# patrikhuber/superviseddescent

Measured on NVIDIA H100. Metric: faces/sec RCR 22-landmark detect, higher is better.
Workload: dtype f32

## Files before the change

superviseddescent_b200/csrc/sd_hog.cu:

```cuda
#include "sd_internal.cuh"
#include "sd_hog_common.cuh"

#include <cmath>
#include <cuda_pipeline.h>

namespace {

constexpr int kHogThreads = 256;

struct HogArgs {
    const uint8_t* images;
    int width, height, row_stride;
    long long image_stride;
    int image_count;
    const int* image_index;
    const sd_roi* roi;
    const sd_frame* frames;
    uint8_t* roi_miss;
    const float* x;
    long long ldx;
    int N, L;
    int variant, nc, cs, K, fs, dd;
    const int* half;
    HogOrient orient;
    const int* rtab;
    const float* btab;
    int tma_count;
    float* A;
    long long ld;
    int* geometry;
    uint8_t* patches;
    int8_t* bins;
    int* status;
};

__device__ __forceinline__ int clip_index(int x, int a, int b) { return x >= a ? (x < b ? x : b - 1) : a; }
__device__ __forceinline__ short sat_short(int v) { return (short)(v > 32767 ? 32767 : (v < -32768 ? -32768 : v)); }

__global__ void hog_geometry_kernel(const float* __restrict__ x, long long ldx, int N, int L, const sd_eyes_dev eyes, float rel,
                                    int fixed_half, int fs, int* __restrict__ half_out, int* __restrict__ rtab, int* __restrict__ status)
{
    const int i = blockIdx.x;
    if (i >= N) return;
    __shared__ int s_half;
    if (threadIdx.x == 0) {
        bool degenerate;
        const int half = sd_patch_half(x + (long long)i * ldx, L, eyes, rel, fixed_half, &degenerate);
        if (degenerate) atomicOr(status, 1);
        half_out[i] = half;
        s_half = half;
    }
    __syncthreads();
    const int P = 2 * s_half;
    int* rt = rtab + (long long)i * 5 * fs;
    for (int t = threadIdx.x; t < fs; t += blockDim.x) {
        const double inv_scale = __ddiv_rn((double)fs, (double)P);
        const double scale = __ddiv_rn(1.0, inv_scale);
        float f = (float)__dadd_rn(__dmul_rn((double)t + 0.5, scale), -0.5);
        const int s = (int)floorf(f);
        f = __fsub_rn(f, (float)s);
        int sx = s;
        float fx = f;
        if (sx < 0) { fx = 0.f; sx = 0; }
        if (sx >= P - 1) { fx = 0.f; sx = P - 1; }
        const short2 xa = make_short2(sat_short(__float2int_rn(__fmul_rn(__fsub_rn(1.f, fx), 2048.f))),
                                      sat_short(__float2int_rn(__fmul_rn(fx, 2048.f))));
        const short2 yb = make_short2(sat_short(__float2int_rn(__fmul_rn(__fsub_rn(1.f, f), 2048.f))),
                                      sat_short(__float2int_rn(__fmul_rn(f, 2048.f))));
        rt[t] = sx;
        rt[fs + t] = *reinterpret_cast<const int*>(&xa);
        rt[2 * fs + t] = clip_index(s, 0, P);
        rt[3 * fs + t] = clip_index(s + 1, 0, P);
        rt[4 * fs + t] = *reinterpret_cast<const int*>(&yb);
    }
}

__global__ void hog_bintab_kernel(int fs, int nc, int cs, float* __restrict__ btab)
{
    __shared__ int s_sbin[256];
    for (int t = threadIdx.x; t < fs; t += blockDim.x) {
        int b;
        float w1, w2;
        hog_spatial_weight(t, cs, &b, &w1, &w2);
        s_sbin[t] = b;
        for (int c = 0; c < nc; ++c) btab[c * fs + t] = (b == c) ? w1 : ((b == c - 1) ? w2 : 0.f);
    }
    __syncthreads();
    int* lohi = reinterpret_cast<int*>(btab + nc * fs);
    for (int c = threadIdx.x; c < nc; c += blockDim.x) {
        int lo = fs, hi = -1;
        for (int t = 1; t <= fs - 2; ++t) {
            const int b = s_sbin[t];
            if (b == c || b == c - 1) { if (t < lo) lo = t; hi = t; }
        }
        lohi[c] = lo;
        lohi[nc + c] = hi;
    }
}

__device__ __forceinline__ int hog_resize_out(int yb, int t0, int t1)
{
    return (((((int)(short)yb) * (t0 >> 4)) >> 16) + (((yb >> 16) * (t1 >> 4)) >> 16) + 2) >> 2;
}

__device__ __forceinline__ int byte_of(unsigned lo, unsigned hi, int n) { return (int)(((n < 4 ? lo : hi) >> (8 * (n & 3))) & 0xffu); }

struct HogSmem {
    int patch, bin, r1, tab, xa, wcell, lo, hi, vote, mbar, stage_end, total;
    int pp;
    int pb, pm;
    int tpad;
};

__host__ __device__ inline int align_up(int v, int a) { return (v + a - 1) / a * a; }

__host__ __device__ inline HogSmem hog_smem_layout(int fs, int nc, int K)
{
    HogSmem s;
    s.pp = align_up(fs, 4);
    s.pm = align_up(fs - 2, 4) + 1;
    s.pb = s.pm - 1;
    if ((s.pb & 7) == 0 && (fs - 2) * (s.pb + 4) <= fs * fs) s.pb += 4;
    int o = 0;
    s.patch = o;
    o = align_up(s.pp * fs, 16);
    s.tab = o;    o += fs * 16;
    s.xa = o;     o += fs * 4;
    s.wcell = o;  o += nc * fs * 4;
    s.lo = o;     o += nc * 4;
    s.hi = o;     o += nc * 4;
    s.mbar = align_up(o, 8); o = s.mbar + 8;
    o = align_up(o, 128);
    s.bin = o;    o = align_up(o + fs * fs, 16);
    s.r1 = o;     o = align_up(o + fs * fs * 4, 16);
    s.tpad = align_up((fs - 2) * nc, 32);
    s.vote = o;
    o += 2 * K * s.tpad * 4;
    s.stage_end = o;
    s.total = align_up(o + 8, 16);
    return s;
}

constexpr int kTmaClasses = 8;
__host__ __device__ constexpr int hog_tma_box(int c) { return c == 0 ? 32 : c == 1 ? 48 : c == 2 ? 64 : c == 3 ? 80 : c == 4 ? 96 : c == 5 ? 112 : c == 6 ? 128 : 160; }
struct HogMaps { CUtensorMap m[kTmaClasses]; };

template <int KT, int NCT, int CST, int NT>
__global__ void __launch_bounds__(NT, NCT > 0 ? 2048 / NT : 0) hog_patch_kernel(const __grid_constant__ HogArgs a, const __grid_constant__ HogMaps maps)
{
    static_assert(NT % 32 == 0 && NT >= 64, "hog_patch_kernel needs whole warps and at least 64 threads");
    constexpr int kWarps = NT / 32;
    extern __shared__ __align__(128) unsigned char smem[];
    const int K = KT > 0 ? KT : a.K;
    const int nc = NCT > 0 ? NCT : a.nc;
    const int fs = (NCT > 0 && CST > 0) ? NCT * CST : a.fs;
    const int cells = nc * nc;
    const HogSmem lay = hog_smem_layout(fs, nc, K);
    const int pp = lay.pp, pb = lay.pb, pm = lay.pm;
    uint8_t* s_patch = smem + lay.patch;
    int8_t* s_bin = reinterpret_cast<int8_t*>(smem + lay.bin);
    float* s_gmag = reinterpret_cast<float*>(smem + lay.r1);
    int4* s_tab = reinterpret_cast<int4*>(smem + lay.tab);
    short2* s_xa = reinterpret_cast<short2*>(smem + lay.xa);
    float* s_wcell = reinterpret_cast<float*>(smem + lay.wcell);
    int* s_lo = reinterpret_cast<int*>(smem + lay.lo);
    int* s_hi = reinterpret_cast<int*>(smem + lay.hi);
    float* s_T = reinterpret_cast<float*>(smem + lay.vote);
    uint64_t* s_mbar = reinterpret_cast<uint64_t*>(smem + lay.mbar);

    const int tid = threadIdx.x;
    const int lane = tid & 31, warp = tid >> 5;
    const long long patch_id = blockIdx.x;
    const int sample = (int)(patch_id / a.L);
    const int lm = (int)(patch_id - (long long)sample * a.L);

    const float* __restrict__ row = a.x + (long long)sample * a.ldx;
    const int half = __ldg(a.half + sample);
    const int P = 2 * half;
    const int cx = __float2int_rn(row[lm]);
    const int cy = __float2int_rn(row[lm + a.L]);
    int img_idx = a.image_index ? a.image_index[sample] : sample;
    if (img_idx < 0 || img_idx >= a.image_count) {
        img_idx = 0;
        if (tid == 0 && a.status) atomicOr(a.status, 2);
    }
    int W = a.width, H = a.height, rs = a.row_stride;
    const uint8_t* __restrict__ img = a.images + (long long)img_idx * a.image_stride;
    if (a.frames) {
        const sd_frame f = a.frames[img_idx];
        W = f.width; H = f.height; rs = f.row_stride;
        img = a.images + f.offset;
    }
    int rx = 0, ry = 0, rw = W, rh = H;
    if (a.roi) {
        const sd_roi r = a.roi[img_idx];
        rx = r.x; ry = r.y; rw = r.w; rh = r.h; rs = r.row_stride;
        img = a.images + r.offset;
    }
    if (tid == 0 && a.geometry) {
        a.geometry[patch_id * 3 + 0] = cx;
        a.geometry[patch_id * 3 + 1] = cy;
        a.geometry[patch_id * 3 + 2] = half;
    }

    const int x0 = cx - half, y0 = cy - half;
    uint8_t* s_stage = smem + lay.bin;
    const int stage_cap = lay.stage_end - lay.bin;
    int tma_box = 0;
    const int tma_shift = x0 & 15;
#pragma unroll
    for (int c = kTmaClasses - 1; c >= 0; --c)
        if (c < a.tma_count && hog_tma_box(c) >= P + tma_shift && hog_tma_box(c) * hog_tma_box(c) <= stage_cap) tma_box = hog_tma_box(c);
    if (tma_box > 0 && tid == 0) {
        int cls = 0;
#pragma unroll
        for (int c = 0; c < kTmaClasses; ++c) if (hog_tma_box(c) == tma_box) cls = c;
        hog_tma_load(s_mbar, s_stage, &maps.m[cls], x0 - tma_shift, y0, img_idx, tma_box * tma_box);
    }

    {
        const int* __restrict__ rt = a.rtab + (long long)sample * 5 * fs;
        for (int t = tid; t < fs; t += NT) {
            const int xa = __ldg(rt + fs + t);
            s_xa[t] = *reinterpret_cast<const short2*>(&xa);
            s_tab[t] = make_int4(__ldg(rt + t), __ldg(rt + 2 * fs + t), __ldg(rt + 3 * fs + t), __ldg(rt + 4 * fs + t));
        }
        for (int i = tid; i < nc * fs; i += NT) s_wcell[i] = __ldg(a.btab + i);
        const int* __restrict__ lohi = reinterpret_cast<const int*>(a.btab + nc * fs);
        if (tid < nc) { s_lo[tid] = __ldg(lohi + tid); s_hi[tid] = __ldg(lohi + nc + tid); }
    }
    {
        const bool resident = x0 >= rx && y0 >= ry && x0 + P <= rx + rw && y0 + P <= ry + rh && x0 >= 0 && y0 >= 0 && x0 + P <= W && y0 + P <= H;
        const uintptr_t align_bits = reinterpret_cast<uintptr_t>(img) | (uintptr_t)rs;
        const bool vec16 = !tma_box && resident && (align_bits & 15) == 0;
        const bool words = !tma_box && resident && (align_bits & 3) == 0;
        const int shiftb = tma_box ? tma_shift : (vec16 ? ((x0 - rx) & 15) : (words ? ((x0 - rx) & 3) : 0));
        const int pitch = tma_box ? tma_box : ((P + 15 + 15) & ~15);
        const bool staged = pitch * P <= stage_cap;
        bool miss = false;
        if (staged) {
            if (tma_box) {
            } else if (vec16) {
                const int nvec = (shiftb + P + 15) >> 4;
                const int gs = nvec <= 8 ? 3 : (nvec <= 16 ? 4 : 5);
                const int lv = lane & ((1 << gs) - 1), lr = lane >> gs, rows_per_pass = 32 >> gs;
                const uint8_t* wrow = img + (long long)(y0 - ry) * rs + (x0 - rx - shiftb);
                for (int r = warp * rows_per_pass + lr; r < P; r += kWarps * rows_per_pass)
#pragma unroll 1
                    for (int v = lv; v < nvec; v += (1 << gs))
                        reinterpret_cast<uint4*>(s_stage + r * pitch)[v] = __ldg(reinterpret_cast<const uint4*>(wrow + (long long)r * rs) + v);
            } else if (words) {
                const int nwords = (shiftb + P + 3) >> 2;
                const uint8_t* wrow = img + (long long)(y0 - ry) * rs + (x0 - rx - shiftb);
                for (int r = warp; r < P; r += kWarps) {
                    const uint32_t* src = reinterpret_cast<const uint32_t*>(wrow + (long long)r * rs);
                    uint32_t* dst = reinterpret_cast<uint32_t*>(s_stage + r * pitch);
#pragma unroll 1
                    for (int w = lane; w < nwords; w += 32) dst[w] = __ldg(src + w);
                }
            } else {
                for (int r = warp; r < P; r += kWarps) {
                    const int iy = y0 + r;
                    const bool rowin = (unsigned)iy < (unsigned)H;
                    const bool rowres = iy >= ry && iy < ry + rh;
                    for (int c = lane; c < P; c += 32) {
                        const int ix = x0 + c;
                        int v = 0;
                        if (rowin && (unsigned)ix < (unsigned)W) {
                            if (rowres && ix >= rx && ix < rx + rw) v = __ldg(img + (long long)(iy - ry) * rs + (ix - rx));
                            else miss = true;
                        }
                        s_stage[r * pitch + c] = (uint8_t)v;
                    }
                }
            }
            __syncthreads();
            if (tma_box) hog_tma_wait(s_mbar);
            if (fs <= 64) {
                const int np = (fs + 1) >> 1, groups = NT / np;
                const int j = tid % np, g = tid / np;
                if (g < groups) {
                    const int dxa = 2 * j, dxb = min(dxa + 1, fs - 1);
                    const int sxa = s_tab[dxa].x, sxb = s_tab[dxb].x;
                    const unsigned xa = *reinterpret_cast<const unsigned*>(s_xa + dxa), xb = *reinterpret_cast<const unsigned*>(s_xa + dxb);
                    const int q = (shiftb + sxa) & ~3;
                    const int oa = shiftb + sxa - q, ob = shiftb + sxb - q;
                    uint8_t* out = s_patch + dxa;
                    if (ob <= 6) {
                        const unsigned sa = oa | (oa + 1) << 4, sb = ob | (ob + 1) << 4;
                        const uint8_t* base = s_stage + q;
#pragma unroll 2
                        for (int dy = g; dy < fs; dy += groups) {
                            const int4 yt = s_tab[dy];
                            const unsigned* r0 = reinterpret_cast<const unsigned*>(base + yt.y * pitch);
                            const unsigned* r1 = reinterpret_cast<const unsigned*>(base + yt.z * pitch);
                            const unsigned a0 = r0[0], a1 = r0[1], b0 = r1[0], b1 = r1[1];
                            const int va = hog_resize_out(yt.w, __dp2a_lo(xa, __byte_perm(a0, a1, sa), 0u), __dp2a_lo(xa, __byte_perm(b0, b1, sa), 0u));
                            const int vb = hog_resize_out(yt.w, __dp2a_lo(xb, __byte_perm(a0, a1, sb), 0u), __dp2a_lo(xb, __byte_perm(b0, b1, sb), 0u));
                            *reinterpret_cast<uint16_t*>(out + dy * pp) = (uint16_t)(va | vb << 8);
                        }
                    } else {
                        const int ax = s_xa[dxa].x, bx = s_xa[dxa].y, cx = s_xa[dxb].x, dx = s_xa[dxb].y;
                        const int sxa1 = min(sxa + 1, P - 1), sxb1 = min(sxb + 1, P - 1);
                        const uint8_t* base = s_stage + shiftb;
                        for (int dy = g; dy < fs; dy += groups) {
                            const int4 yt = s_tab[dy];
                            const uint8_t* r0 = base + yt.y * pitch;
                            const uint8_t* r1 = base + yt.z * pitch;
                            const int va = hog_resize_out(yt.w, (int)r0[sxa] * ax + (int)r0[sxa1] * bx, (int)r1[sxa] * ax + (int)r1[sxa1] * bx);
                            const int vb = hog_resize_out(yt.w, (int)r0[sxb] * cx + (int)r0[sxb1] * dx, (int)r1[sxb] * cx + (int)r1[sxb1] * dx);
                            *reinterpret_cast<uint16_t*>(out + dy * pp) = (uint16_t)(va | vb << 8);
                        }
                    }
                }
            } else {
                for (int dy = warp; dy < fs; dy += kWarps) {
                    const int4 yt = s_tab[dy];
                    const uint8_t* r0 = s_stage + yt.y * pitch + shiftb;
                    const uint8_t* r1 = s_stage + yt.z * pitch + shiftb;
                    for (int dx = lane; dx < fs; dx += 32) {
                        const int sx = s_tab[dx].x;
                        const int sx1 = min(sx + 1, P - 1);
                        const short2 xa = s_xa[dx];
                        const int t0 = (int)r0[sx] * xa.x + (int)r0[sx1] * xa.y;
                        const int t1 = (int)r1[sx] * xa.x + (int)r1[sx1] * xa.y;
                        s_patch[dy * pp + dx] = (uint8_t)hog_resize_out(yt.w, t0, t1);
                    }
                }
            }
        } else {
            __syncthreads();
            for (int dy = warp; dy < fs; dy += kWarps) {
                const int4 yt = s_tab[dy];
                const int iy0 = y0 + yt.y, iy1 = y0 + yt.z;
                for (int dx = lane; dx < fs; dx += 32) {
                    const int sx = s_tab[dx].x;
                    const short2 xa = s_xa[dx];
                    int p[4];
#pragma unroll
                    for (int q = 0; q < 4; ++q) {
                        const int ix = x0 + sx + (q & 1), iy = (q & 2) ? iy1 : iy0;
                        int v = 0;
                        if ((q & 1) && xa.y == 0) { p[q] = 0; continue; }
                        if ((unsigned)ix < (unsigned)W && (unsigned)iy < (unsigned)H) {
                            if (ix >= rx && ix < rx + rw && iy >= ry && iy < ry + rh) v = __ldg(img + (long long)(iy - ry) * rs + (ix - rx));
                            else miss = true;
                        }
                        p[q] = v;
                    }
                    const int t0 = p[0] * xa.x + p[1] * xa.y;
                    const int t1 = p[2] * xa.x + p[3] * xa.y;
                    s_patch[dy * pp + dx] = (uint8_t)hog_resize_out(yt.w, t0, t1);
                }
            }
        }
        if (miss && a.roi_miss) a.roi_miss[img_idx] = 1;
        if (a.patches) {
            __syncthreads();
            for (int i = tid; i < fs * fs; i += NT) {
                const int y = i / fs;
                a.patches[patch_id * fs * fs + i] = s_patch[y * pp + (i - y * fs)];
            }
        }
    }
    __syncthreads();

    {
        const int iw = fs - 2, runs = (iw + 3) >> 2, nitem = iw * runs;
        const int pw = pp >> 2;
        for (int i = tid; i < nitem; i += NT) {
            const int y = i / runs, r = i - y * runs;
            const unsigned* c = reinterpret_cast<const unsigned*>(s_patch) + (y + 1) * pw + r;
            const unsigned c0 = c[0], c1 = c[1], u0 = c[-pw], u1 = c[1 - pw], d0 = c[pw], d1 = c[pw + 1];
            unsigned bins = 0;
            float* gm = s_gmag + y * pm + 4 * r;
#pragma unroll
            for (int k = 0; k < 4; ++k) {
                const int gx = byte_of(c0, c1, k + 2) - byte_of(c0, c1, k);
                const int gy = byte_of(d0, d1, k + 1) - byte_of(u0, u1, k + 1);
                const int g2 = gx * gx + gy * gy;
                const float g = __fsqrt_rn((float)g2);
                const int b = hog_bin(a.orient, K, gx, gy, g);
                bins |= (unsigned)(b & 0xff) << (8 * k);
                gm[k] = b < 0 ? 0.f : g;
            }
            *reinterpret_cast<unsigned*>(s_bin + y * pb + 4 * r) = bins;
        }
    }
    if (a.bins) {
        __syncthreads();
        for (int idx = tid; idx < fs * fs; idx += NT) {
            const int y = idx / fs, x = idx - y * fs;
            const bool interior = x >= 1 && x <= fs - 2 && y >= 1 && y <= fs - 2;
            a.bins[patch_id * fs * fs + idx] = interior ? s_bin[(y - 1) * pb + x - 1] : (int8_t)-1;
        }
    }
    if (!a.A) return;
    __syncthreads();

    {
        const int nrow = fs - 2, ntask = nrow * nc, tpad = lay.tpad;
        for (int task = tid; task < ntask; task += NT) {
            const int ci = task / nrow, y = 1 + task - ci * nrow;
            const int xlo = s_lo[ci], xhi = s_hi[ci];
            const int8_t* bp = s_bin + (y - 1) * pb + (xlo - 1);
            const float* gp = s_gmag + (y - 1) * pm + (xlo - 1);
            const float* wp = s_wcell + ci * fs + xlo;
            float* T = s_T + task;
            for (int b = 0; b < 2 * K; ++b) T[b * tpad] = 0.f;
#pragma unroll 2
            for (int x = xlo; x <= xhi; ++x) {
                const int b = max((int)*bp++, 0);
                float* q = T + b * tpad;
                *q = __fadd_rn(*q, __fmul_rn(*gp++, *wp++));
            }
        }
        __syncthreads();
        float* __restrict__ out = a.A + (long long)sample * a.ld + (long long)lm * cells * a.dd;
        for (int i = tid; i < 2 * K * cells; i += NT) {
            const int b = i / cells, c = i - b * cells;
            const int cj = c / nc, ci = c - cj * nc;
            const int ylo = s_lo[cj], yhi = s_hi[cj];
            const float* Tp = s_T + b * tpad + ci * nrow + (ylo - 1);
            const float* wy = s_wcell + cj * fs + ylo;
            float acc = 0.f;
            for (int y = ylo; y <= yhi; ++y) acc = __fadd_rn(acc, __fmul_rn(*Tp++, *wy++));
            out[i] = acc;
        }
    }
}

struct NormArgs {
    float* A;
    long long ld;
    int N, L, nc, K, dd, variant, per_cta;
};

__host__ __device__ inline int hog_norm_smem(int nc, int K, int per_cta)
{
    const int cells = nc * nc;
    return per_cta * (8 + 2 * K * cells * 4 + cells * 8 + (nc + 1) * (nc + 1) * 8);
}

template <int KT>
__global__ void __launch_bounds__(kHogThreads) hog_normalise_kernel(const NormArgs a)
{
    extern __shared__ __align__(16) unsigned char s_norm[];
    const int K = KT > 0 ? KT : a.K;
    const int nc = a.nc, nb = nc + 1, cells = nc * nc, blocks = nb * nb, hsz = 2 * K * cells, per_lm = cells * a.dd;
    const long long first = (long long)blockIdx.x * a.per_cta;
    const int np = (int)min((long long)a.per_cta, (long long)a.N * a.L - first);
    long long* s_slice = reinterpret_cast<long long*>(s_norm);
    double* s_energy = reinterpret_cast<double*>(s_slice + a.per_cta);
    double* s_fac = s_energy + a.per_cta * cells;
    float* s_hist = reinterpret_cast<float*>(s_fac + a.per_cta * blocks);
    for (int p = threadIdx.x; p < np; p += kHogThreads) {
        const long long id = first + p;
        const int sample = (int)(id / a.L), lm = (int)(id - (long long)sample * a.L);
        s_slice[p] = (long long)sample * a.ld + (long long)lm * per_lm;
        if (lm == 0) a.A[(long long)sample * a.ld + (long long)a.L * per_lm] = 1.0f;
    }
    __syncthreads();
    for (int i = threadIdx.x; i < np * hsz; i += kHogThreads) {
        const int p = i / hsz;
        __pipeline_memcpy_async(s_hist + i, a.A + s_slice[p] + (i - p * hsz), sizeof(float));
    }
    __pipeline_commit();
    __pipeline_wait_prior(0);
    __syncthreads();
    for (int i = threadIdx.x; i < np * cells; i += kHogThreads) {
        const int p = i / cells, c = i - p * cells;
        s_energy[i] = (double)hog_cell_energy(s_hist + p * hsz + c, cells, K);
    }
    __syncthreads();
    for (int i = threadIdx.x; i < np * blocks; i += kHogThreads) {
        const int p = i / blocks, j = i - p * blocks;
        const int jy = j / nb, jx = j - jy * nb;
        s_fac[i] = hog_block_factor(s_energy + p * cells, nc, max(jx - 1, 0), min(jx, nc - 1), max(jy - 1, 0), min(jy, nc - 1));
    }
    __syncthreads();
    for (int i = threadIdx.x; i < np * cells; i += kHogThreads) {
        const int p = i / cells, c = i - p * cells;
        const int cj = c / nc, ci = c - cj * nc;
        const double* F = s_fac + p * blocks + cj * nb + ci;
        const double fac[4] = {F[0], F[1], F[nb], F[nb + 1]};
        float* __restrict__ out = a.A + s_slice[p] + ci * nc + cj;
        hog_cell_features(fac, s_hist + p * hsz + c, cells, K, a.variant, [=](int d, float v) { out[d * cells] = v; });
    }
}

int launch_hog(sd_ctx* ctx, const sd_image_batch* images, const int32_t* d_image_index, const float* d_x,
               int64_t ldx, int N, int L, const sd_normalisation* eyes, const sd_hog_param* p, float* d_A,
               int64_t ld, int32_t* d_geometry, uint8_t* d_patches, int8_t* d_bins)
{
    SD_REQUIRE(ctx, images && images->d_data && d_x && p, "null argument");
    SD_REQUIRE(ctx, N >= 0 && L >= 1, "bad sample / landmark count");
    SD_REQUIRE(ctx, p->variant == 0 || p->variant == 1, "unknown HOG variant");
    SD_REQUIRE(ctx, p->num_bins >= 1 && p->num_bins <= SD_MAX_BINS, "num_bins must be in [1,16]");
    SD_REQUIRE(ctx, p->num_cells >= 1 && p->cell_size >= 1, "bad cell configuration");
    const int fs = p->num_cells * p->cell_size;
    SD_REQUIRE(ctx, fs > 3 && fs <= 256, "resized patch must be 4..256 px (hog.c:545-546 asserts > 3)");
    SD_REQUIRE(ctx, (fs + p->cell_size / 2) / p->cell_size == p->num_cells, "hogWidth != num_cells");
    SD_REQUIRE(ctx, ldx >= 2 * L, "ldx < 2L");
    if (N == 0) return SD_OK;
    const bool fixed = !eyes || eyes->kind == 0;
    int fixed_half = 0;
    if (fixed) {
        fixed_half = p->num_cells * (p->cell_size / 2);
        SD_REQUIRE(ctx, 2 * fixed_half == fs, "the fixed-patch HogTransform needs an even cell_size (patch == num_cells * cell_size)");
    } else if (eyes->kind != 1) {
        return sd_fail(ctx, SD_ERR_INVALID, "unknown normalisation kind");
    }

    HogArgs a;
    sd_eyes_dev eyes_dev;
    memset(&eyes_dev, 0, sizeof(eyes_dev));
    int rc = fixed ? SD_OK : sd_eyes_to_dev(ctx, eyes, L, &eyes_dev);
    if (rc) return rc;
    a.images = images->d_data;
    a.width = images->width; a.height = images->height; a.row_stride = images->row_stride;
    a.image_stride = images->image_stride; a.image_count = images->count;
    a.image_index = d_image_index;
    a.roi = images->d_roi;
    a.roi_miss = images->d_roi_miss;
    a.frames = images->d_frames;
    if (!d_image_index) SD_REQUIRE(ctx, images->count >= N, "fewer images than samples and no image index");
    a.x = d_x; a.ldx = ldx; a.N = N; a.L = L;
    a.variant = p->variant; a.nc = p->num_cells; a.cs = p->cell_size; a.K = p->num_bins; a.fs = fs;
    a.dd = p->variant == 1 ? 3 * p->num_bins + 4 : 4 * p->num_bins;
    a.A = d_A; a.ld = ld;
    if (d_A) SD_REQUIRE(ctx, ld >= (int64_t)L * a.nc * a.nc * a.dd + 1, "ld < feature length");
    const HogSmem lay = hog_smem_layout(fs, a.nc, a.K);
    const int cells = a.nc * a.nc;
    NormArgs na;
    na.A = d_A; na.ld = ld; na.N = N; na.L = L; na.nc = a.nc; na.K = a.K; na.dd = a.dd; na.variant = a.variant;
    na.per_cta = cells < kHogThreads ? kHogThreads / cells : 1;
    const int norm_smem = hog_norm_smem(a.nc, a.K, na.per_cta);
    SD_REQUIRE(ctx, lay.total <= 227 * 1024 && norm_smem <= 227 * 1024, "HOG configuration needs more than 227 KB of shared memory");
    const long long blocks = (long long)N * L;
    SD_REQUIRE(ctx, blocks < 2147483647LL, "too many patches for one launch");
    a.geometry = d_geometry; a.patches = d_patches; a.bins = d_bins;
    a.status = reinterpret_cast<int*>(ctx->d_scratch) + 1;

    hog_orientations(a.K, a.orient);

    const size_t geom_bytes = (size_t)N * sizeof(int) + (size_t)N * 5 * fs * sizeof(int) + (size_t)(a.nc * fs + 2 * a.nc) * sizeof(float);
    int* d_half = (int*)sd_workspace(ctx, SD_WS_GEOM, geom_bytes);
    if (!d_half) return SD_ERR_CUDA;
    int* d_rtab = d_half + N;
    float* d_btab = reinterpret_cast<float*>(d_rtab + (size_t)N * 5 * fs);
    hog_geometry_kernel<<<N, 64, 0, ctx->stream>>>(d_x, ldx, N, L, eyes_dev, p->relative_patch_size, fixed_half, fs, d_half, d_rtab, a.status);
    SD_LAUNCH_CHECK(ctx, "hog_geometry_kernel");
    hog_bintab_kernel<<<1, 256, 0, ctx->stream>>>(fs, a.nc, a.cs, d_btab);
    SD_LAUNCH_CHECK(ctx, "hog_bintab_kernel");
    a.half = d_half;
    a.rtab = d_rtab;
    a.btab = d_btab;

    HogMaps maps;
    memset(&maps, 0, sizeof(maps));
    a.tma_count = 0;
    if (!images->d_roi && (images->image_stride % 16) == 0 && (images->count == 1 || images->image_stride > 0)) {
        for (int c = 0; c < kTmaClasses && hog_tma_box(c) <= 256; ++c) {
            if (!hog_frame_map(images, hog_tma_box(c), hog_tma_box(c), &maps.m[c])) break;
            a.tma_count = c + 1;
        }
    }

    auto kern = hog_patch_kernel<0, 0, 0, kHogThreads>;
    int threads = kHogThreads;
    if (a.K == 4) kern = hog_patch_kernel<4, 0, 0, kHogThreads>;
    else if (a.K == 9) kern = hog_patch_kernel<9, 0, 0, kHogThreads>;
    if (a.nc == 5 && (a.K == 4 || a.K == 9)) {
#define SD_HOG_PICK(KK, CC, TT) if (a.K == KK && a.cs == CC) { kern = hog_patch_kernel<KK, 5, CC, TT>; threads = TT; }
        SD_HOG_PICK(4, 11, 224) SD_HOG_PICK(4, 10, 160) SD_HOG_PICK(4, 8, 160) SD_HOG_PICK(4, 6, 128)
        SD_HOG_PICK(9, 11, 256) SD_HOG_PICK(9, 10, 160) SD_HOG_PICK(9, 8, 160) SD_HOG_PICK(9, 6, 128)
#undef SD_HOG_PICK
    }
    SD_CUDA(ctx, cudaFuncSetAttribute(kern, cudaFuncAttributeMaxDynamicSharedMemorySize, lay.total));
    kern<<<(unsigned)blocks, threads, lay.total, ctx->stream>>>(a, maps);
    SD_LAUNCH_CHECK(ctx, "hog_patch_kernel");
    if (!d_A) return SD_OK;
    auto norm = a.K == 4 ? hog_normalise_kernel<4> : a.K == 9 ? hog_normalise_kernel<9> : hog_normalise_kernel<0>;
    SD_CUDA(ctx, cudaFuncSetAttribute(norm, cudaFuncAttributeMaxDynamicSharedMemorySize, norm_smem));
    norm<<<(unsigned)sd_div_up(blocks, na.per_cta), kHogThreads, norm_smem, ctx->stream>>>(na);
    SD_LAUNCH_CHECK(ctx, "hog_normalise_kernel");
    return SD_OK;
}

}

namespace {
__global__ void bgr2gray_kernel(const uint8_t* __restrict__ bgr, int width, int height, long long srow, long long simg, int count,
                                uint8_t* __restrict__ gray, long long drow, long long dimg, int vec_ok)
{
    const int groups = (width + 3) >> 2;
    const long long total = (long long)count * height * groups;
    for (long long t = blockIdx.x * (long long)blockDim.x + threadIdx.x; t < total; t += (long long)gridDim.x * blockDim.x) {
        const int g = (int)(t % groups);
        const long long ry = t / groups;
        const int y = (int)(ry % height);
        const long long im = ry / height;
        const uint8_t* s = bgr + im * simg + (long long)y * srow + 12 * g;
        uint8_t* d = gray + im * dimg + (long long)y * drow + 4 * g;
        const int x0 = 4 * g;
        if (vec_ok && x0 + 4 <= width) {
            const uint32_t w0 = *reinterpret_cast<const uint32_t*>(s), w1 = *reinterpret_cast<const uint32_t*>(s + 4),
                           w2 = *reinterpret_cast<const uint32_t*>(s + 8);
            const uint32_t b0 = w0 & 255, g0 = (w0 >> 8) & 255, r0 = (w0 >> 16) & 255, b1 = w0 >> 24;
            const uint32_t g1 = w1 & 255, r1 = (w1 >> 8) & 255, b2 = (w1 >> 16) & 255, g2 = w1 >> 24;
            const uint32_t r2 = w2 & 255, b3 = (w2 >> 8) & 255, g3 = (w2 >> 16) & 255, r3 = w2 >> 24;
            const uint32_t y0 = sd_bgr_to_gray(b0, g0, r0), y1 = sd_bgr_to_gray(b1, g1, r1);
            const uint32_t y2 = sd_bgr_to_gray(b2, g2, r2), y3 = sd_bgr_to_gray(b3, g3, r3);
            *reinterpret_cast<uint32_t*>(d) = y0 | (y1 << 8) | (y2 << 16) | (y3 << 24);
        } else {
            for (int k = 0; k < 4 && x0 + k < width; ++k) d[k] = (uint8_t)sd_bgr_to_gray(s[3 * k], s[3 * k + 1], s[3 * k + 2]);
        }
    }
}
}

extern "C" {

int sd_hog_feature_length(int num_landmarks, const sd_hog_param* p)
{
    if (!p) return -1;
    const int dd = p->variant == 1 ? 3 * p->num_bins + 4 : 4 * p->num_bins;
    return num_landmarks * p->num_cells * p->num_cells * dd + 1;
}

int sd_hog_batch(sd_ctx* ctx, const sd_image_batch* images, const int32_t* d_image_index, const float* d_x,
                 int64_t ldx, int num_samples, int num_landmarks, const sd_normalisation* eyes,
                 const sd_hog_param* p, float* d_A, int64_t ld)
{
    if (!ctx) return SD_ERR_INVALID;
    if (num_samples == 0) return SD_OK;
    SD_REQUIRE(ctx, d_A, "null output");
    return launch_hog(ctx, images, d_image_index, d_x, ldx, num_samples, num_landmarks, eyes, p, d_A, ld,
                      nullptr, nullptr, nullptr);
}

int sd_hog_debug(sd_ctx* ctx, const sd_image_batch* images, const int32_t* d_image_index, const float* d_x,
                 int64_t ldx, int num_samples, int num_landmarks, const sd_normalisation* eyes,
                 const sd_hog_param* p, int32_t* d_geometry, uint8_t* d_patches, int8_t* d_bins)
{
    if (!ctx) return SD_ERR_INVALID;
    return launch_hog(ctx, images, d_image_index, d_x, ldx, num_samples, num_landmarks, eyes, p, nullptr, 0,
                      d_geometry, d_patches, d_bins);
}

int sd_bgr2gray(sd_ctx* ctx, const uint8_t* d_bgr, int width, int height, int64_t bgr_row_stride, int64_t bgr_image_stride,
                int count, uint8_t* d_gray, int64_t gray_row_stride, int64_t gray_image_stride)
{
    if (!ctx) return SD_ERR_INVALID;
    SD_REQUIRE(ctx, count >= 0 && width > 0 && height > 0, "bad argument");
    if (count == 0) return SD_OK;
    SD_REQUIRE(ctx, d_bgr && d_gray && bgr_row_stride >= 3LL * width && gray_row_stride >= width, "bad argument");
    const int vec_ok = ((reinterpret_cast<uintptr_t>(d_bgr) | reinterpret_cast<uintptr_t>(d_gray) | (uintptr_t)bgr_row_stride |
                         (uintptr_t)bgr_image_stride | (uintptr_t)gray_row_stride | (uintptr_t)gray_image_stride) & 3) == 0;
    const long long total = (long long)count * height * ((width + 3) >> 2);
    const int blocks = (int)(sd_div_up(total, 256) < 16LL * ctx->sm_count ? sd_div_up(total, 256) : 16LL * ctx->sm_count);
    bgr2gray_kernel<<<blocks, 256, 0, ctx->stream>>>(d_bgr, width, height, bgr_row_stride, bgr_image_stride, count, d_gray,
                                                     gray_row_stride, gray_image_stride, vec_ok);
    SD_LAUNCH_CHECK(ctx, "bgr2gray_kernel");
    return SD_OK;
}

}
```

Measured before the change: 807,600.

## Vectorize HOG histogram voting with 4-wide aligned bin, magnitude and weight rows

Re-lays out the spatial weight table, bin buffer and gradient magnitude buffer in shared memory so rows are padded and aligned to 4 interior pixels. The per-row voting loop then reads packed 4-byte bins, float2 magnitudes and float4 weights, processing four pixels per iteration, with zero-padded weights covering the extra lanes. Gradient writes are packed as float2 stores. This aims to cut shared-memory load instructions in the voting loop, at the cost of a more intricate layout, some wasted work on padding pixels, and possible new bank conflicts.

Result: faster. 823,500, median of 6 (+2.0%).

```diff
diff --git a/superviseddescent_b200/csrc/sd_hog.cu b/superviseddescent_b200/csrc/sd_hog.cu
--- a/superviseddescent_b200/csrc/sd_hog.cu
+++ b/superviseddescent_b200/csrc/sd_hog.cu
@@ -78,15 +78,19 @@
 __global__ void hog_bintab_kernel(int fs, int nc, int cs, float* __restrict__ btab)
 {
     __shared__ int s_sbin[256];
+    const int pi = (fs + 1) & ~3;
     for (int t = threadIdx.x; t < fs; t += blockDim.x) {
         int b;
         float w1, w2;
         hog_spatial_weight(t, cs, &b, &w1, &w2);
         s_sbin[t] = b;
-        for (int c = 0; c < nc; ++c) btab[c * fs + t] = (b == c) ? w1 : ((b == c - 1) ? w2 : 0.f);
-    }
-    __syncthreads();
-    int* lohi = reinterpret_cast<int*>(btab + nc * fs);
+        if (t >= 1 && t <= fs - 2)
+            for (int c = 0; c < nc; ++c) btab[c * pi + t - 1] = (b == c) ? w1 : ((b == c - 1) ? w2 : 0.f);
+    }
+    for (int c = threadIdx.x; c < nc; c += blockDim.x)
+        for (int j = fs - 2; j < pi; ++j) btab[c * pi + j] = 0.f;
+    __syncthreads();
+    int* lohi = reinterpret_cast<int*>(btab + nc * pi);
     for (int c = threadIdx.x; c < nc; c += blockDim.x) {
         int lo = fs, hi = -1;
         for (int t = 1; t <= fs - 2; ++t) {
@@ -108,6 +112,7 @@
 struct HogSmem {
     int patch, bin, r1, tab, xa, wcell, lo, hi, vote, mbar, stage_end, total;
     int pp;
+    int pi;
     int pb, pm;
     int tpad;
 };
@@ -117,22 +122,28 @@
 __host__ __device__ inline HogSmem hog_smem_layout(int fs, int nc, int K)
 {
     HogSmem s;
+    const int iw = fs - 2;
     s.pp = align_up(fs, 4);
-    s.pm = align_up(fs - 2, 4) + 1;
-    s.pb = s.pm - 1;
-    if ((s.pb & 7) == 0 && (fs - 2) * (s.pb + 4) <= fs * fs) s.pb += 4;
+    s.pi = align_up(iw, 4);
+    s.pm = align_up(iw, 2);
+    if ((s.pm & 3) == 0) s.pm += 2;
     int o = 0;
     s.patch = o;
     o = align_up(s.pp * fs, 16);
     s.tab = o;    o += fs * 16;
+    s.wcell = o;  o += nc * s.pi * 4;
     s.xa = o;     o += fs * 4;
-    s.wcell = o;  o += nc * fs * 4;
     s.lo = o;     o += nc * 4;
     s.hi = o;     o += nc * 4;
     s.mbar = align_up(o, 8); o = s.mbar + 8;
     o = align_up(o, 128);
-    s.bin = o;    o = align_up(o + fs * fs, 16);
-    s.r1 = o;     o = align_up(o + fs * fs * 4, 16);
+    s.bin = o;
+    const int span_end = align_up(align_up(o + fs * fs, 16) + fs * fs * 4, 16);
+    const int mod_bytes = ((iw - 1) * s.pm + s.pi) * 4;
+    s.pb = s.pi;
+    if ((s.pb & 4) == 0 && align_up(o + (iw - 1) * (s.pb + 4) + s.pi, 16) + mod_bytes <= span_end) s.pb += 4;
+    s.r1 = align_up(o + (iw - 1) * s.pb + s.pi, 16);
+    o = span_end;
     s.tpad = align_up((fs - 2) * nc, 32);
     s.vote = o;
     o += 2 * K * s.tpad * 4;
@@ -156,7 +167,7 @@
     const int fs = (NCT > 0 && CST > 0) ? NCT * CST : a.fs;
     const int cells = nc * nc;
     const HogSmem lay = hog_smem_layout(fs, nc, K);
-    const int pp = lay.pp, pb = lay.pb, pm = lay.pm;
+    const int pp = lay.pp, pi = lay.pi, pb = lay.pb, pm = lay.pm;
     uint8_t* s_patch = smem + lay.patch;
     int8_t* s_bin = reinterpret_cast<int8_t*>(smem + lay.bin);
     float* s_gmag = reinterpret_cast<float*>(smem + lay.r1);
@@ -225,8 +236,8 @@
             s_xa[t] = *reinterpret_cast<const short2*>(&xa);
             s_tab[t] = make_int4(__ldg(rt + t), __ldg(rt + 2 * fs + t), __ldg(rt + 3 * fs + t), __ldg(rt + 4 * fs + t));
         }
-        for (int i = tid; i < nc * fs; i += NT) s_wcell[i] = __ldg(a.btab + i);
-        const int* __restrict__ lohi = reinterpret_cast<const int*>(a.btab + nc * fs);
+        for (int i = tid; i < nc * pi; i += NT) s_wcell[i] = __ldg(a.btab + i);
+        const int* __restrict__ lohi = reinterpret_cast<const int*>(a.btab + nc * pi);
         if (tid < nc) { s_lo[tid] = __ldg(lohi + tid); s_hi[tid] = __ldg(lohi + nc + tid); }
     }
     {
@@ -366,14 +377,14 @@
     __syncthreads();
 
     {
-        const int iw = fs - 2, runs = (iw + 3) >> 2, nitem = iw * runs;
+        const int iw = fs - 2, runs = pi >> 2, nitem = iw * runs;
         const int pw = pp >> 2;
         for (int i = tid; i < nitem; i += NT) {
             const int y = i / runs, r = i - y * runs;
             const unsigned* c = reinterpret_cast<const unsigned*>(s_patch) + (y + 1) * pw + r;
             const unsigned c0 = c[0], c1 = c[1], u0 = c[-pw], u1 = c[1 - pw], d0 = c[pw], d1 = c[pw + 1];
             unsigned bins = 0;
-            float* gm = s_gmag + y * pm + 4 * r;
+            float m[4];
 #pragma unroll
             for (int k = 0; k < 4; ++k) {
                 const int gx = byte_of(c0, c1, k + 2) - byte_of(c0, c1, k);
@@ -382,9 +393,12 @@
                 const float g = __fsqrt_rn((float)g2);
                 const int b = hog_bin(a.orient, K, gx, gy, g);
                 bins |= (unsigned)(b & 0xff) << (8 * k);
-                gm[k] = b < 0 ? 0.f : g;
+                m[k] = b < 0 ? 0.f : g;
             }
             *reinterpret_cast<unsigned*>(s_bin + y * pb + 4 * r) = bins;
+            float2* gm = reinterpret_cast<float2*>(s_gmag + y * pm + 4 * r);
+            gm[0] = make_float2(m[0], m[1]);
+            if (4 * r + 2 < pm || y == iw - 1) gm[1] = make_float2(m[2], m[3]);
         }
     }
     if (a.bins) {
@@ -403,16 +417,25 @@
         for (int task = tid; task < ntask; task += NT) {
             const int ci = task / nrow, y = 1 + task - ci * nrow;
             const int xlo = s_lo[ci], xhi = s_hi[ci];
-            const int8_t* bp = s_bin + (y - 1) * pb + (xlo - 1);
-            const float* gp = s_gmag + (y - 1) * pm + (xlo - 1);
-            const float* wp = s_wcell + ci * fs + xlo;
+            const int j0 = (xlo - 1) & ~3;
+            const int8_t* bp = s_bin + (y - 1) * pb + j0;
+            const float* gp = s_gmag + (y - 1) * pm + j0;
+            const float* wp = s_wcell + ci * pi + j0;
             float* T = s_T + task;
             for (int b = 0; b < 2 * K; ++b) T[b * tpad] = 0.f;
-#pragma unroll 2
-            for (int x = xlo; x <= xhi; ++x) {
-                const int b = max((int)*bp++, 0);
-                float* q = T + b * tpad;
-                *q = __fadd_rn(*q, __fmul_rn(*gp++, *wp++));
+            const auto vote = [&](unsigned byte, float g, float w) {
+                float* q = T + min(byte & 0xffu, 2u * K - 1u) * tpad;
+                *q = __fadd_rn(*q, __fmul_rn(g, w));
+            };
+            for (int x = j0 + 1; x <= xhi; x += 4) {
+                const unsigned bw = *reinterpret_cast<const unsigned*>(bp);
+                const float2 g01 = *reinterpret_cast<const float2*>(gp), g23 = *reinterpret_cast<const float2*>(gp + 2);
+                const float4 w = *reinterpret_cast<const float4*>(wp);
+                bp += 4; gp += 4; wp += 4;
+                vote(bw, g01.x, w.x);
+                vote(bw >> 8, g01.y, w.y);
+                vote(bw >> 16, g23.x, w.z);
+                vote(bw >> 24, g23.y, w.w);
             }
         }
         __syncthreads();
@@ -422,7 +445,7 @@
             const int cj = c / nc, ci = c - cj * nc;
             const int ylo = s_lo[cj], yhi = s_hi[cj];
             const float* Tp = s_T + b * tpad + ci * nrow + (ylo - 1);
-            const float* wy = s_wcell + cj * fs + ylo;
+            const float* wy = s_wcell + cj * pi + (ylo - 1);
             float acc = 0.f;
             for (int y = ylo; y <= yhi; ++y) acc = __fadd_rn(acc, __fmul_rn(*Tp++, *wy++));
             out[i] = acc;
@@ -544,7 +567,7 @@
 
     hog_orientations(a.K, a.orient);
 
-    const size_t geom_bytes = (size_t)N * sizeof(int) + (size_t)N * 5 * fs * sizeof(int) + (size_t)(a.nc * fs + 2 * a.nc) * sizeof(float);
+    const size_t geom_bytes = (size_t)N * sizeof(int) + (size_t)N * 5 * fs * sizeof(int) + (size_t)(a.nc * lay.pi + 2 * a.nc) * sizeof(float);
     int* d_half = (int*)sd_workspace(ctx, SD_WS_GEOM, geom_bytes);
     if (!d_half) return SD_ERR_CUDA;
     int* d_rtab = d_half + N;
```
